# zhengpuas47/ImageAnalysis3

Hardware: AMD Instinct MI355X
Metric: fitted spots/sec (+ FOVs/sec), 2048x2048x50 float32 stack, ~5k spots/FOV (higher is better)
Workload: dtype f64

## Files before the change

### imageanalysis3_amd/csrc/fit.hip

```cpp
#include "ia3_rt.h"
#include "ia3_lm.h"
#include "ia3_init.h"
#include "ia3_kdtree.h"
#include <algorithm>
#include <numeric>
#include <math.h>
#include <string.h>
#include <stddef.h>
#include <time.h>
#include <stdio.h>
#include <stdlib.h>
#include <unistd.h>
#include <mutex>

using namespace ia3;

namespace ia3k {
void kd_build(const double* points, int n, std::vector<ia3::KdNode>& nodes, std::vector<int>& indices, double* mins,
              double* maxes);
}

namespace {

constexpr int SLOTS = 8;
// ... 779 lines not shown
    success_old = LDH(&fa.state[i].success);
    co0 = LDH(&fa.ps[(size_t)i * 11 + 1]); co1 = LDH(&fa.ps[(size_t)i * 11 + 2]); co2 = LDH(&fa.ps[(size_t)i * 11 + 3]);
  }
  const bool ok = n >= NP;
  int nfev = 0, nfev_first = 0;
  const int npass = mode == 2 ? 2 : 1;
#pragma unroll 1
  for (int pass = 0; pass < npass; ++pass) {
    const bool refit = mode == 1 || pass == 1;
    if (pass == 1) { success_old = ok ? 1 : 0; co0 = L->p[1]; co1 = L->p[2]; co2 = L->p[3]; nfev_first = nfev; }
    if (ok) nfev = wave_gaussfit(fa, L, valid, refit ? 2 : (fa.dtype == IA3_F32 ? 0 : 1), c0,
                                 refit ? fa.delta_repeat : fa.delta_first, n, mode == 2 && pass == 0);
  }
  if (mode == 2 && ok && (threadIdx.x & 63) == 0) L->tally[0] += 1ull;
  bool cv = true;
  if (mode != 0 && ok && success_old) {
    const float d0 = co0 - L->p[1], d1 = co1 - L->p[2], d2 = co2 - L->p[3];
    const float dist = (d0 * d0 + d1 * d1) + d2 * d2;
    cv = (double)dist < fa.dist_th2;
  }
  store_result(fa, i, L, mode == 0 ? fa.delta_first : fa.delta_repeat, ok, n, nfev + nfev_first, mode != 0, cv);
  IA3_STAMP(L, 11);
  return cv;
}

constexpr int NCLAIM = 8;
struct StageCtl {
  int n_unconv;
  int abort;
  int ties;
  int stage_reached;
  int pad[28];
  struct Claim { unsigned int next; unsigned int pad[31]; } claim[NCLAIM + 1];
};
static_assert(sizeof(StageCtl) == 128 * (NCLAIM + 2), "one 128-byte line per counter");

__device__ long long d_wait_bound = 1LL << 22;

__device__ __forceinline__ bool wait_done(const int* done, int j, int need, StageCtl* ctl) {
  long long spins = 0;
  for (;;) {
    const int v = __builtin_amdgcn_readfirstlane(__hip_atomic_load(&done[j], __ATOMIC_RELAXED, __HIP_MEMORY_SCOPE_AGENT));
    if (v >= need) { if (spins) __builtin_amdgcn_s_setprio(3); return true; }
    if (spins == 0) __builtin_amdgcn_s_setprio(0);
    if (spins < 256) __builtin_amdgcn_s_sleep(16);
    else if (spins < 1024) __builtin_amdgcn_s_sleep(64);
    else { __builtin_amdgcn_s_sleep(127); __builtin_amdgcn_s_sleep(127); }
    ++spins;
    if ((spins & 15) == 0) {
      const int ab = __builtin_amdgcn_readfirstlane(__hip_atomic_load(&ctl->abort, __ATOMIC_RELAXED, __HIP_MEMORY_SCOPE_AGENT));
      if (spins > d_wait_bound || ab) {
        __hip_atomic_store(&ctl->abort, 1, __ATOMIC_RELAXED, __HIP_MEMORY_SCOPE_AGENT);
        return false;
      }
    }
  }
}

__device__ __forceinline__ void publish(int* done, int i, int value) {
  if ((threadIdx.x & 63) == 0) {
    __builtin_amdgcn_fence(__ATOMIC_RELEASE, "agent");
    asm volatile("s_waitcnt vmcnt(0)" ::: "memory");
    __hip_atomic_fetch_max(&done[i], value, __ATOMIC_RELAXED, __HIP_MEMORY_SCOPE_AGENT);
  }
}

__device__ __forceinline__ void publish_quiet(int* done, int i, int value) {
  if ((threadIdx.x & 63) == 0) __hip_atomic_fetch_max(&done[i], value, __ATOMIC_RELAXED, __HIP_MEMORY_SCOPE_AGENT);
// ... 258 lines not shown
  bool pristine;
  bool first_done;
  StageCtl host_ctl;
  unsigned long long host_counters[5];
  void *d_tie_flag, *d_tie_lost;
  void* kd_block;
  bool ties_resolved;
  bool ties_host = false;
  std::vector<double> host_seeds;
  std::vector<char> kd_stage;
  bool cached;
  std::vector<char> host_stage;
  void* d_snap = nullptr;
};

namespace {

int build_ball(int r, std::vector<signed char>& ball) {
  ball.clear();
  for (int z = -r; z < r; ++z)
    for (int x = -r; x < r; ++x)
      for (int y = -r; y < r; ++y)
        if (z * z + x * x + y * y <= r * r) { ball.push_back((signed char)z); ball.push_back((signed char)x); ball.push_back((signed char)y); ball.push_back(0); }
  return (int)(ball.size() / 4);
}

int g_nb_cap = MAXNB;
int g_fit_fuse = 1;
int g_fit_maxfev = 0;
int g_fit_waves = 2;
int g_fit_merge = 1;
int g_fit_memo = 1;
int g_fit_kdq = KDQ_CAP;

FitArgs make_args(const ia3_fitter* f) {
  FitArgs a;
  a.ims = (const void* const*)f->d_ims; a.fov_of = (const int*)f->d_fov_of; a.fov_start = (const int*)f->d_fov_start;
  a.n_fov = (int)f->ims.size(); a.fov_counters = (unsigned long long*)f->d_fov_counters;
  a.dtype = f->im->dtype; a.Z = f->im->Z; a.X = f->im->X; a.Y = f->im->Y;
  a.n = f->n; a.fuse = g_fit_fuse; a.nb_cap = g_nb_cap; a.nb_r2 = 4.0 * f->prm.radius_fit * (double)f->prm.radius_fit;
  a.seeds = (const double*)f->d_seeds; a.nbr_cnt = (const int*)f->d_nbr_cnt; a.nbr_idx = (const int*)f->d_nbr_idx;
  a.ball = (const int*)f->d_ball; a.nball = f->nball; a.radius = f->prm.radius_fit;
  a.tie_lost = f->ties_resolved ? (const unsigned long long*)f->d_tie_lost : nullptr;
  a.state = (SeedState*)f->d_state; a.ps = (float*)f->d_ps; a.nvox = (int*)f->d_nvox; a.nfev = (int*)f->d_nfev;
  a.memo = g_fit_memo ? (unsigned long long*)f->d_memo : nullptr;
  a.conv = (unsigned char*)f->d_conv; a.n_iter = (int*)f->d_niter; a.counters = (unsigned long long*)f->d_counters;
  a.min_ws = f->prm.min_w * f->prm.min_w; a.max_ws = f->prm.max_w * f->prm.max_w; a.init_w = f->prm.init_w;
  a.delta_first = f->prm.min_delta_center; a.delta_repeat = f->prm.max_delta_center;
  a.dist_th2 = f->prm.max_dist_th * f->prm.max_dist_th;
  a.n_max_iter = f->prm.n_max_iter;
  a.ftol = 1.49012e-8; a.xtol = 1.49012e-8; a.gtol = 0.0; a.maxfev = 1000; a.factor = 100.0;
  if (f->prm.model_variant == 1) {
    a.maxfev = 100 * (NP + 1);
    a.variant = 1;
    for (int k = 0; k < 3; ++k) {
      double w = f->prm.init_w_zxy[k];
      if (w * w > f->prm.max_w || w * w < f->prm.min_w) w = 1.5 * 1.5;
      a.iw[k] = log((a.max_ws - w * w) / (w * w - a.min_ws));
    }
  }
  if (g_fit_maxfev > 0) a.maxfev = g_fit_maxfev;
  return a;
}

}

// ... 162 lines not shown
                       (unsigned long long*)f->d_fov_counters);
  }
  {
    hipError_t le = hipGetLastError();
    if (le != hipSuccess) { ia3_fit_destroy(f); return set_error(IA3_EHIP, "fitter setup launch failed: %s", hipGetErrorString(le)); }
  }
  *out = f;
  return IA3_OK;
}

int ia3_fit_create(const ia3_stack* im, const double* centers_zxy, int n, const ia3_fit_params* p,
                   ia3_fitter** out) {
  if (!im || n < 0 || (n > 0 && !centers_zxy)) return set_error(IA3_EINVAL, "bad argument");
  const FovSeeds one{im, centers_zxy, nullptr, n};
  return fit_create_impl(&one, 1, p, out);
}

}

namespace ia3k {
void set_fit_nblist(int cap) { g_nb_cap = cap < 0 ? 0 : (cap > MAXNB ? MAXNB : cap); }
int get_fit_nblist() { return g_nb_cap; }
void set_fit_fuse(int on) { g_fit_fuse = on ? 1 : 0; }
void set_fit_maxfev(int n) { g_fit_maxfev = n; }
void set_fit_waves(int n) { g_fit_waves = n < 1 ? 1 : (n > IA3_FIT_LB ? IA3_FIT_LB : n); }
void set_fit_merge(int on) { g_fit_merge = on != 0; }
int set_fit_waitbound(int polls) {
  int rc = ia3rt::ensure_init(); if (rc) return rc;
  const long long v = polls > 0 ? (long long)polls : (1LL << 22);
  IA3_HIP(hipMemcpyToSymbol(HIP_SYMBOL(d_wait_bound), &v, sizeof(v)));
  return IA3_OK;
}
void set_fit_memo(int on) { g_fit_memo = on != 0; }
void set_fit_kdq(int cap) { g_fit_kdq = cap < 1 ? 1 : (cap > KDQ_CAP ? KDQ_CAP : cap); }
void fit_host_counters(const ia3_fitter* f, long long out[5]) {
  for (int k = 0; k < 5; ++k) out[k] = (long long)f->host_counters[k];
}
int fit_create_dev(const ia3_stack* im, const double* d_centers_zxy, int n, const ia3_fit_params* p, ia3_fitter** out) {
  if (!im || n < 0 || (n > 0 && !d_centers_zxy)) return set_error(IA3_EINVAL, "bad argument");
  const FovSeeds one{im, nullptr, d_centers_zxy, n};
  return fit_create_impl(&one, 1, p, out);
}
int fit_create_ahead(const ia3_stack* im, const double* d_centers_zxy, int capacity, const unsigned* d_count, int n_cut,
                     const ia3_fit_params* p, ia3_fitter** out) {
  if (!im || capacity < 1 || !d_centers_zxy || !d_count) return set_error(IA3_EINVAL, "bad argument");
  const FovSeeds one{im, nullptr, d_centers_zxy, capacity};
  return fit_create_impl(&one, 1, p, out, d_count, n_cut);
}
int fit_set_count(ia3_fitter* f, int n) {
  if (!f || n < 0 || n > f->n || f->ims.size() != 1) return set_error(IA3_EINVAL, "bad seed count");
  f->n = n;
  f->fov_start.assign({0, n});
  return IA3_OK;
}
int fit_max_fovs() { return MAX_FOV; }
int fit_create_multi(const ia3_stack* const* ims, const double* const* d_centers_zxy, const int* n_seeds, int n_fov,
                     const ia3_fit_params* p, ia3_fitter** out) {
  std::vector<FovSeeds> v((size_t)(n_fov > 0 ? n_fov : 0));
  for (int k = 0; k < n_fov; ++k) v[(size_t)k] = FovSeeds{ims[k], nullptr, d_centers_zxy[k], n_seeds[k]};
  return fit_create_impl(v.data(), n_fov, p, out);
}
int fit_fov_results(ia3_fitter* f, int* n_iter, long long* counters3) {
  const int nf = (int)f->ims.size();
  std::vector<int> it((size_t)nf);
  std::vector<unsigned long long> c(4 * (size_t)nf);
  IA3_HIP(hipStreamSynchronize(stream()));
// ... 15 lines not shown
  hipStream_t st = stream();
  if (fresh) {
    if (!f->pristine) {
      memset(&f->host_ctl, 0, sizeof(StageCtl));
      f->host_ctl.n_unconv = f->n;
      static_assert(offsetof(StageCtl, n_unconv) == 0 && offsetof(StageCtl, abort) == 4, "the first two words are re-armed together");
      IA3_HIP(hipMemcpyAsync(f->d_ctl, &f->host_ctl, 2 * sizeof(int), hipMemcpyHostToDevice, st));
    }
  }
  if (!fresh || !f->pristine)
    IA3_HIP(hipMemsetAsync((char*)f->d_ctl + offsetof(StageCtl, claim), 0, sizeof(StageCtl) - offsetof(StageCtl, claim), st));
  f->pristine = false;
  long long blocks = (long long)(stage1 - stage0) * f->n;
  const long long simds = 4LL * num_cus() * g_fit_waves;
  if (blocks > simds) blocks = simds;
  if (blocks < 1) blocks = 1;
  ProfScope ps(stage0 == 0 ? "fit_first" : "fit_repeat");
  hipLaunchKernelGGL(fit_stages_k, dim3((unsigned)blocks), dim3(64), 0, st, a, f->n, stage0, stage1, (StageCtl*)f->d_ctl,
                     (int*)f->d_done);
  dbg_stamp("fit_stages launched");
  IA3_KCHECK();
  return IA3_OK;
}


__global__ __launch_bounds__(1024) void mail_copy_k(const unsigned* __restrict__ src, unsigned* __restrict__ dst, size_t n4,
                                                    volatile unsigned* seq_word, unsigned seq) {
  const size_t n16 = n4 / 4;
  for (size_t i = threadIdx.x; i < n16; i += 1024) ((uint4*)dst)[i] = ((const uint4*)src)[i];
  for (size_t i = 4 * n16 + threadIdx.x; i < n4; i += 1024) dst[i] = src[i];
  __threadfence_system();
  __syncthreads();
  if (threadIdx.x == 0) *seq_word = seq;
}
static int fetch_block(ia3_fitter* f, bool with_rows) {
  hipStream_t st = stream();
  const size_t head = (size_t)((char*)f->d_ps - (char*)f->d_counters);
  const size_t rows = with_rows ? sizeof(float) * 11 * (size_t)f->n : 0;
  f->host_stage.resize(head + rows);
  void *mh = nullptr, *md = nullptr;
  constexpr size_t MAIL_OFF = 4096;
  constexpr size_t SEQ_OFF = 2048;
  static_assert(sizeof(uint4) == 16, "");
  if (head + rows <= (1u << 20) - MAIL_OFF && (head + rows) % 4 == 0 && ((size_t)f->d_counters & 15) == 0 &&
      host_mailbox(1u << 20, &mh, &md) == IA3_OK) {
    static thread_local unsigned t_seq = 0;
    const unsigned seq = ++t_seq ? t_seq : ++t_seq;
    hipLaunchKernelGGL(mail_copy_k, dim3(1), dim3(1024), 0, st, (const unsigned*)f->d_counters, (unsigned*)((char*)md + MAIL_OFF),
                       (head + rows) / 4, (volatile unsigned*)((char*)md + SEQ_OFF), seq);
    IA3_KCHECK();
    ws_put_deferred_now();
    volatile unsigned* mb = (volatile unsigned*)((char*)mh + SEQ_OFF);
    SpinWait sw;
    while (*mb != seq) {
      sw.relax();
      if (((sw.n & 0xfffff) == 0 || (sw.n > 40400 && (sw.n & 0x3ff) == 0)) && hipStreamQuery(st) != hipErrorNotReady) {
        if (*mb == seq) break;
        IA3_HIP(hipStreamSynchronize(st));
        if (*mb != seq) return set_error(IA3_EHIP, "fit results did not reach the host mailbox");
        break;
      }
    }
    memcpy(f->host_stage.data(), (char*)mh + MAIL_OFF, head + rows);
    return IA3_OK;
  }
  { int rc = stream_wait_spin(st); if (rc) return rc; }
  IA3_HIP(hipMemcpyAsync(f->host_stage.data(), f->d_counters, head + rows, hipMemcpyDeviceToHost, st));
  IA3_HIP(hipStreamSynchronize(st));
  return IA3_OK;
}

static int resolve_ties_host(ia3_fitter* f);
static int resolve_ties(ia3_fitter* f) {
  hipStream_t st = stream();
  const int n = f->n, nf = (int)f->ims.size();
  std::vector<int> flagged((size_t)nf, 1);
  if (f->host_seeds.empty()) {
    f->host_seeds.resize(3 * (size_t)n);
    IA3_HIP(hipMemcpyAsync(f->host_seeds.data(), f->d_seeds, sizeof(double) * 3 * (size_t)n, hipMemcpyDeviceToHost, st));
  }
  IA3_HIP(hipMemcpyAsync(flagged.data(), f->d_fov_ties, sizeof(int) * (size_t)nf, hipMemcpyDeviceToHost, st));
  IA3_HIP(hipStreamSynchronize(st));
// ... 558 lines not shown
```

### imageanalysis3_amd/csrc/gauss.hip

```cpp
#include "ia3_gauss.h"
#include <unistd.h>
#include <cstring>
#include <mutex>

using namespace ia3g;

namespace {

__global__ void border_map_k(int* bmap, int count, int R, int len, int mode) {
  int i = blockIdx.x * 256 + threadIdx.x;
  if (i < count) bmap[i] = border_idx(i - R, len, mode);
}

template <class T, int R, int K, bool TR = false>
__global__ __launch_bounds__(256) void gauss_strided(const T* __restrict__ in, T* __restrict__ out,
                                                     int inner, size_t stride, int len,
                                                     size_t outer_stride, Taps taps,
                                                     const int* __restrict__ bmap, int seg, int cert) {
  constexpr bool FAST = R >= 16;
  constexpr int TQ = (K == 6 || K == 12) ? 24 : ((K == 10) ? 30 : 32);
  static_assert(!TR || TQ % K == 0, "tile must hold whole chunks");
  __shared__ float tile[TR ? 4 : 1][TR ? 64 : 1][TR ? TQ + 1 : 1];
  const int p_raw = blockIdx.x * 256 + threadIdx.x;
  if (!TR && p_raw >= inner) return;
// ... 732 lines not shown
}

using namespace ia3rt;

extern "C" {

int ia3_prepare_depth(int dtype, int Z) {
  int rc = ensure_init(); if (rc) return rc;
  if (dtype != IA3_F32 && dtype != IA3_U16) return set_error(IA3_EINVAL, "dtype");
  return ia3g::column_kernel_source(dtype == IA3_F32, Z);
}
int ia3_set_tuning(int key, int value) {
  if (key == IA3_TUNE_GAUSS_CERT) {
    if (value < -2) return set_error(IA3_EINVAL, "IA3_TUNE_GAUSS_CERT: value must be >= -2");
    g_cert = value;
    return 0;
  }
  if (key == IA3_TUNE_GAUSS_FOLD) { g_fold_on = value != 0; return 0; }
  if (key == IA3_TUNE_DFT_VALU) { ia3k::set_dft_valu(value); return 0; }
  if (key == IA3_TUNE_UPLOAD_THREADS) return ia3rt::set_upload_threads(value);
  if (key == IA3_TUNE_SEED_DENSE) { ia3k::set_seed_dense(value); return 0; }
  if (key == IA3_TUNE_SEED_STRIPS) { ia3k::set_seed_strips(value); return 0; }
  if (key == IA3_TUNE_SEED_FUSED) { ia3k::set_seed_fused(value); return 0; }
  if (key == IA3_TUNE_SEED_SKIP) { ia3k::set_seed_skip(value); return 0; }
  if (key == IA3_TUNE_FIT_NBLIST) { ia3k::set_fit_nblist(value); return 0; }
  if (key == IA3_TUNE_FFT_C2C) { ia3k::set_fft_c2c(value); return 0; }
  if (key == IA3_TUNE_FIT_FUSE) { ia3k::set_fit_fuse(value); return 0; }
  if (key == IA3_TUNE_FIT_WAVES) { ia3k::set_fit_waves(value); return 0; }
  if (key == IA3_TUNE_FIT_MERGE) { ia3k::set_fit_merge(value); return 0; }
  if (key == IA3_TUNE_WARP_ONEPASS) { ia3k::set_warp_onepass(value); return 0; }
  if (key == IA3_TUNE_FIT_KDQ) { ia3k::set_fit_kdq(value); return 0; }
  if (key == IA3_TUNE_FIT_MEMO) { ia3k::set_fit_memo(value); return 0; }
  if (key == IA3_TUNE_COL_RTC) { ia3g::set_column_rtc(value != 0); return 0; }
  if (key == IA3_DEBUG_FIT_MAXFEV) { ia3k::set_fit_maxfev(value); return 0; }
  if (key == IA3_DEBUG_FIT_WAITBOUND) return ia3k::set_fit_waitbound(value);
  return set_error(IA3_EINVAL, "unknown tuning key");
}

static int taps_or_default(double sigma, double truncate, const double* weights, int radius,
                           std::vector<double>& w, int& R) {
  if (weights) {
    if (radius < 0) return set_error(IA3_EINVAL, "negative radius");
    w.assign(weights, weights + 2 * radius + 1);
    R = radius;
  } else {
    if (!(sigma > 0)) return set_error(IA3_EINVAL, "sigma must be > 0");
    gaussian_taps(sigma, truncate, w, R);
  }
  return IA3_OK;
}

int ia3_gaussian_filter_dev(const ia3_stack* im, double sigma, double truncate, int mode,
                            const double* weights, int radius, ia3_stack* out) {
  int rc = ensure_init(); if (rc) return rc;
  if (!im || !out) return set_error(IA3_EINVAL, "null stack");
  if (im->dtype != out->dtype || im->Z != out->Z || im->X != out->X || im->Y != out->Y)
    return set_error(IA3_EINVAL, "input/output stacks differ in shape or dtype");
  if (mode != IA3_MODE_REFLECT && mode != IA3_MODE_NEAREST) return set_error(IA3_EUNSUPPORTED, "mode %d", mode);
  std::vector<double> w; int R;
  rc = taps_or_default(sigma, truncate, weights, radius, w, R); if (rc) return rc;
  Scratch tmp(im->bytes);
  if (!tmp.p) return IA3_ENOMEM;
  if (im->d == out->d) return set_error(IA3_EINVAL, "in-place filtering is not supported");
  return ia3k::gaussian3d(im->d, im->dtype, im->Z, im->X, im->Y, w.data(), R, mode, out->d, tmp.p);
}

// ... 41 lines not shown
```

### imageanalysis3_amd/csrc/ia3_rt.h

```cpp
#pragma once
#include <hip/hip_runtime.h>
#include <stdint.h>
#include <stddef.h>
#include <string>
#include <vector>
#include "../../include/ia3.h"

struct ia3_stack {
  void* d;
  int dtype, Z, X, Y;
  bool owned;
  size_t bytes;
  void* home = nullptr;
};

namespace ia3rt {

int set_error(int code, const char* fmt, ...);
int ensure_init();
hipStream_t stream();
int num_cus();
int host_mailbox(size_t bytes, void** host, void** dev);
int stream_wait_spin(hipStream_t st);
struct SpinWait {
// ... 37 lines not shown
                              hipGetErrorString(_e), __FILE__, __LINE__);                  \
  } while (0)

struct AuxScope {
  bool ok;
  AuxScope();
  ~AuxScope();
};
struct AuxResume {
  bool ok;
  AuxResume();
  ~AuxResume();
};
int aux_join();
struct PutDefer {
  bool outer;
  PutDefer();
  ~PutDefer();
};
void ws_put_deferred_now();
void dbg_stamp(const char* what);

struct ProfScope {
  int slot;
  explicit ProfScope(const char* name);
  ~ProfScope();
};

void gaussian_taps(double sigma, double truncate, std::vector<double>& w, int& radius);

}

namespace ia3k { void set_dft_valu(int on); void set_fft_c2c(int on); void set_seed_dense(int on);
void set_seed_strips(int on); void set_seed_fused(int on); void set_seed_skip(int v); void set_fit_nblist(int cap); void set_fit_fuse(int on); void set_fit_waves(int n); void set_fit_maxfev(int n); void set_fit_merge(int on); void set_warp_onepass(int v); void set_fit_kdq(int cap); void set_fit_memo(int on); int set_fit_waitbound(int polls); }
namespace ia3k {
int gaussian3d(const void* src, int dtype, int Z, int X, int Y, const double* w, int radius, int mode,
               void* dst, void* tmp, int axes = 3);
int highpass_combine(const void* im, const void* low, int dtype, size_t n, void* out);
constexpr int DOG_PAIR_ZGROUPS = 5;
size_t dog_pair_strips(int X, int Y);
int gauss_dog_pair(const void* src, int dtype, int Z, int X, int Y, const double* wf, int rf, const double* wb, int rb,
                   void* dst_front, void* dst_zp, void* tmp, int* forked, float* tmax = nullptr, float* smin = nullptr,
                   float* sabs = nullptr, float* smx = nullptr);
void dog_pair_tiles(int X, int Y, int* ty, int* ntile, size_t* count);
const int* reflect_map(int count, int R, int len);
struct SeedOut {
  std::vector<double> zxyh;
  double th_used;
};
int dog_seed(const ia3_stack* im, const ia3_seed_params& p, SeedOut& out);
struct SeedDev {
  bool on_device = false;
  int n = 0;
  double th_used = 0;
  const double* d_zxy = nullptr;
  const double* d_h = nullptr;
  void* hold = nullptr;
  void (*ahead)(void* ctx, const double* d_zxy, const unsigned* d_count, int max_num_seeds) = nullptr;
  void* ahead_ctx = nullptr;
  SeedOut host;
  ~SeedDev() { if (hold) ia3rt::ws_put(hold); }
};
int dog_seed_dev(const ia3_stack* im, const ia3_seed_params& p, SeedDev& out);
int fit_create_dev(const ia3_stack* im, const double* d_centers_zxy, int n, const ia3_fit_params* p, ia3_fitter** out);
int fit_create_ahead(const ia3_stack* im, const double* d_centers_zxy, int capacity, const unsigned* d_count, int n_cut,
                     const ia3_fit_params* p, ia3_fitter** out);
int fit_set_count(ia3_fitter* f, int n);
// ... 14 lines not shown
```

### imageanalysis3_amd/csrc/seed.hip

```cpp
#include "ia3_rt.h"
#include "ia3_gauss_dev.h"
#include "ia3_seedskip.h"
#include <memory>
#include <algorithm>
#include <math.h>
#include <string.h>
#include <time.h>
#include <stdio.h>
#include <stdlib.h>

namespace {

struct Cand { int z, x, y; float h; };

constexpr int MAXLEV = 64;
struct Levels { double th[MAXLEV]; int n; };

struct SeedCtl {
  unsigned int n_cand;
  unsigned int overflow;
  unsigned int pad[2];
};

template <class T> __device__ __forceinline__ T ldc(const T* p, int z, int x, int y, int X, int Y) {
// ... 791 lines not shown
  __shared__ int chosen_s;
  const unsigned tid = threadIdx.x;
  if (tid < MAXLEV) cnt[tid] = 0;
  if (tid == 0) nk = 0;
  __syncthreads();
  const unsigned n = fin_n(sctl);
  for (unsigned i = tid; i < n; i += 1024) {
    const double h = (double)c[i].h;
    for (int l = 0; l < lev.n; ++l) if (h >= lev.th[l]) atomicAdd(&cnt[l], 1u);
  }
  __syncthreads();
  if (tid == 0) {
    int chosen = lev.n - 1;
    for (int l = 0; l < lev.n; ++l) if ((long long)cnt[l] >= (long long)min_dyn) { chosen = l; break; }
    chosen_s = chosen;
  }
  __syncthreads();
  const double th = lev.th[chosen_s];
  for (unsigned i0 = 0; i0 < n; i0 += 1024) {
    const unsigned i = i0 + tid;
    Cand k{0, 0, 0, 0.f};
    if (i < n) k = c[i];
    const bool keep = i < n && (double)k.h >= th;
    const unsigned long long m = __ballot(keep);
    unsigned base = 0;
    if ((tid & 63) == 0 && m) base = atomicAdd(&nk, (unsigned)__popcll(m));
    base = __shfl(base, 0, 64);
    const unsigned pos = base + (unsigned)__popcll(m & ((1ull << (tid & 63)) - 1ull));
    if (keep && pos < FIN_KEYS) kc[pos] = k;
  }
  __syncthreads();
  const unsigned kept = nk < FIN_KEYS ? nk : FIN_KEYS;
  for (unsigned i = tid; i < kept; i += 1024) { hotcnt[i] = 0u; rank[i] = 0u; }
  if (tid == 0) { fc->chosen = chosen_s; fc->n_kept = nk; fc->n_alive = 0u; fc->done = 0u; }
}
__device__ __forceinline__ unsigned fin_kept(const FinCtl* fc) { return fc->n_kept <= FIN_KEYS ? fc->n_kept : 0u; }

__global__ __launch_bounds__(256) void fin_hot_k(const Cand* __restrict__ kc, const FinCtl* __restrict__ fc, unsigned* __restrict__ hotcnt) {
  __shared__ int tx[256], ty[256];
  const unsigned n = fin_kept(fc);
  if (blockIdx.x * 256 >= n) return;
  const unsigned i = blockIdx.x * 256 + threadIdx.x;
  const int xi = i < n ? kc[i].x : -1, yi = i < n ? kc[i].y : -1;
  const unsigned per = (n + FIN_S - 1) / FIN_S, j0 = blockIdx.y * per, j1 = j0 + per < n ? j0 + per : n;
  unsigned cnt = 0;
  for (unsigned jb = j0; jb < j1; jb += 256) {
    const unsigned j = jb + threadIdx.x;
    __syncthreads();
    tx[threadIdx.x] = j < j1 ? kc[j].x : -2;
    ty[threadIdx.x] = j < j1 ? kc[j].y : -2;
    __syncthreads();
    const unsigned m = j1 - jb < 256 ? j1 - jb : 256;
    for (unsigned t = 0; t < m; ++t) cnt += (tx[t] == xi && ty[t] == yi);
  }
  if (i < n && cnt) atomicAdd(&hotcnt[i], cnt);
}

__global__ __launch_bounds__(256) void fin_rank_k(const Cand* __restrict__ kc, FinCtl* __restrict__ fc, const unsigned* __restrict__ hotcnt,
                                                  int hot_th, unsigned* __restrict__ rank) {
  __shared__ unsigned long long tk[256];
  const unsigned n = fin_kept(fc);
  if (blockIdx.x * 256 >= n) return;
  const unsigned i = blockIdx.x * 256 + threadIdx.x;
  const bool alive = i < n && (hot_th <= 0 || hotcnt[i] < (unsigned)hot_th);
  const unsigned long long ki = i < n ? fin_key(kc[i]) : ~0ull;
  const unsigned per = (n + FIN_S - 1) / FIN_S, j0 = blockIdx.y * per, j1 = j0 + per < n ? j0 + per : n;
  unsigned r = 0;
// ... 4 lines not shown
    tk[threadIdx.x] = aj ? fin_key(kc[j]) : 0ull;
    __syncthreads();
    const unsigned m = j1 - jb < 256 ? j1 - jb : 256;
    for (unsigned t = 0; t < m; ++t) r += tk[t] > ki;
  }
  if (alive) {
    if (r) atomicAdd(&rank[i], r);
    if (blockIdx.y == 0) atomicAdd(&fc->n_alive, 1u);
  }
}

__global__ __launch_bounds__(256) void fin_scatter_k(const SeedCtl* __restrict__ sctl, const Cand* __restrict__ kc, const FinCtl* fc,
                                                     const unsigned* __restrict__ hotcnt, int hot_th, const unsigned* __restrict__ rank,
                                                     int max_num, double* __restrict__ zxy, double* __restrict__ hh, FinCtl* fcw,
                                                     const SeedCtl* __restrict__ lazy, unsigned cap0,
                                                     volatile unsigned* __restrict__ mail, unsigned seq) {
  const unsigned n = fin_kept(fc);
  const unsigned i = blockIdx.x * 256 + threadIdx.x;
  if (i < n) {
    const bool alive = hot_th <= 0 || hotcnt[i] < (unsigned)hot_th;
    const unsigned r = alive ? rank[i] : 0u;
    if (alive && !(max_num > 0 && r >= (unsigned)max_num)) {
      const Cand k = kc[i];
      zxy[3 * r] = k.z; zxy[3 * r + 1] = k.x; zxy[3 * r + 2] = k.y;
      hh[r] = (double)k.h;
    }
  }
  __threadfence();
  __syncthreads();
  if (threadIdx.x != 0) return;
  if (atomicAdd(&fcw->done, 1u) != gridDim.x - 1) return;
  __threadfence();
  const unsigned nc = sctl->n_cand;
  const unsigned ov = sctl->overflow | ((lazy && (lazy->overflow || lazy->n_cand > cap0)) ? 2u : 0u) | (fc->n_kept > FIN_KEYS ? 4u : 0u);
  fcw->n_cand = nc;
  fcw->overflow = ov;
  fcw->pad[0] = lazy ? lazy->pad[0] : 0u;
  if (mail) {
    mail[1] = fcw->n_alive; mail[2] = (unsigned)fcw->chosen; mail[3] = nc; mail[4] = ov;
    mail[5] = fcw->pad[0];
    __threadfence_system();
    mail[0] = seq;
  }
}

}

using namespace ia3rt;

namespace ia3k {

static void finish_seeds(std::vector<Cand>& c, const Levels& lev, const ia3_seed_params& p, int Y,
                         SeedOut& o) {
  int chosen = lev.n - 1;
  for (int i = 0; i < lev.n; ++i) {
    long long cnt = 0;
    for (auto& k : c) cnt += ((double)k.h >= lev.th[i]);
    if (cnt >= (long long)p.min_dynamic_seeds) { chosen = i; break; }
  }
  o.th_used = lev.th[chosen];
  std::vector<Cand> s;
  s.reserve(c.size());
  for (auto& k : c) if ((double)k.h >= lev.th[chosen]) s.push_back(k);
  if (p.remove_hot_pixel && !s.empty()) {
    size_t cap = 64;
    while (cap < 4 * s.size()) cap <<= 1;
    std::vector<long long> keys(cap, -1);
    std::vector<int> cnts(cap, 0);
    auto slot = [&](long long key) {
      size_t h = (size_t)((unsigned long long)key * 0x9E3779B97F4A7C15ull >> 20) & (cap - 1);
      while (keys[h] != -1 && keys[h] != key) h = (h + 1) & (cap - 1);
      return h;
    };
    bool any_hot = false;
    for (auto& k : s) {
      const long long key = (long long)k.x * (Y + 1) + k.y;
      size_t h = slot(key);
      keys[h] = key;
      if (++cnts[h] >= p.hot_pixel_th) any_hot = true;
    }
    if (any_hot) {
      std::vector<Cand> kept;
      kept.reserve(s.size());
      for (auto& k : s) if (cnts[slot((long long)k.x * (Y + 1) + k.y)] < p.hot_pixel_th) kept.push_back(k);
      s.swap(kept);
    }
  }
  std::sort(s.begin(), s.end(), [](const Cand& a, const Cand& b) {
    if (a.h != b.h) return a.h > b.h;
    if (a.z != b.z) return a.z > b.z;
    if (a.x != b.x) return a.x > b.x;
    return a.y > b.y;
  });
  if (p.max_num_seeds > 0 && (size_t)p.max_num_seeds <= s.size()) s.resize(p.max_num_seeds);
  o.zxyh.resize(s.size() * 4);
  for (size_t i = 0; i < s.size(); ++i) {
    o.zxyh[4 * i + 0] = s[i].z; o.zxyh[4 * i + 1] = s[i].x; o.zxyh[4 * i + 2] = s[i].y; o.zxyh[4 * i + 3] = (double)s[i].h;
  }
}

static double now_ms() { struct timespec t; clock_gettime(CLOCK_MONOTONIC, &t); return t.tv_sec * 1e3 + t.tv_nsec * 1e-6; }

int g_strip_bound = 1;
void set_seed_strips(int on) { g_strip_bound = on ? 1 : 0; }
int g_seed_dense = 0;
void set_seed_dense(int on) { g_seed_dense = on ? 1 : 0; }
int g_seed_fused = 1;
void set_seed_fused(int on) { g_seed_fused = on ? 1 : 0; }
int g_seed_skip = 2;
void set_seed_skip(int v) { g_seed_skip = v < 0 ? 0 : (v > 2 ? 2 : v); }
static thread_local double t_skip_run = 0, t_skip_all = 0;

constexpr unsigned LAZY_CAP = 1u << 17;

inline size_t lazy_bound_offset(size_t nb) { return 2 * ((nb + 1) & ~(size_t)1); }
inline double* lazy_bound_ptr(void* bnd, size_t nb) { return (double*)((float*)bnd + lazy_bound_offset(nb)); }
inline size_t lazy_bound_bytes(size_t nb) { return lazy_bound_offset(nb) * sizeof(float) + nb * sizeof(double); }

template <class T>
static void launch_lazy(const void* mx, const void* zp, int Z, int X, int Y, const double* w, int R, int edge,
                        double th_low, void* bnd, Cand0* c0, SeedCtl* ctl0, Cand* out, unsigned capacity, SeedCtl* ctl,
                        hipStream_t s, int stage, const float* smax = nullptr, int sm_ty = 0, int sm_ntile = 0) {
  const int B = R <= 32 ? 32 : 64;
  const int nbx = (X + B - 1) / B, nby = (Y + B - 1) / B;
  const size_t nb = (size_t)Z * nbx * nby;
  float* bmin = (float*)bnd;
  float* babs = bmin + nb;
  double* lb = lazy_bound_ptr(bnd, nb);
  if (stage == 0) {
    ProfScope ps("seed_blockmin");
    constexpr int V = 16 / (int)sizeof(T);
    const bool wide = Y % V == 0 && ((uintptr_t)zp & 15) == 0;
    const int per = 256 * (wide ? V : 1);
    dim3 g((unsigned)((Y + per - 1) / per), (unsigned)nbx, (unsigned)Z);
    if (B == 32 && wide) hipLaunchKernelGGL((blockmin_k<T, 32, V>), g, dim3(256), 0, s, (const T*)zp, Z, X, Y, nbx, nby, bmin, babs);
    else if (B == 32) hipLaunchKernelGGL((blockmin_k<T, 32, 1>), g, dim3(256), 0, s, (const T*)zp, Z, X, Y, nbx, nby, bmin, babs);
    else if (wide) hipLaunchKernelGGL((blockmin_k<T, 64, V>), g, dim3(256), 0, s, (const T*)zp, Z, X, Y, nbx, nby, bmin, babs);
    else hipLaunchKernelGGL((blockmin_k<T, 64, 1>), g, dim3(256), 0, s, (const T*)zp, Z, X, Y, nbx, nby, bmin, babs);
    hipLaunchKernelGGL(blockbound_k, dim3((unsigned)((nb + 255) / 256)), dim3(256), 0, s, (const float*)bmin, (const float*)babs,
// ... 204 lines not shown
    if (fused) {
      const double th_low = th_list;
      const float* sm = (n_strip && g_strip_bound) ? smin_d : nullptr;
      if (im->dtype == IA3_F32) {
        rc = launch_front<float>(tmp2.p, w.data(), Z, X, Y, p.min_edge_distance, th_low, bnd.p, sm, sabs_d, c0buf.as<Cand0>(), dlazy, s, smx_d, skip_sup);
        if (!rc) launch_lazy<float>(nullptr, b.p, Z, X, Y, wb.data(), Rb, p.min_edge_distance, th_low, bnd.p, c0buf.as<Cand0>(), dlazy, dcand, capacity, dctl, s, 2);
      } else {
        rc = launch_front<uint16_t>(tmp2.p, w.data(), Z, X, Y, p.min_edge_distance, th_low, bnd.p, sm, sabs_d, c0buf.as<Cand0>(), dlazy, s, smx_d, skip_sup);
        if (!rc) launch_lazy<uint16_t>(nullptr, b.p, Z, X, Y, wb.data(), Rb, p.min_edge_distance, th_low, bnd.p, c0buf.as<Cand0>(), dlazy, dcand, capacity, dctl, s, 2);
      }
      if (rc) return rc;
    } else if (lazy) {
      if (im->dtype == IA3_F32)
        launch_lazy<float>(maxim, b.p, Z, X, Y, wb.data(), Rb, p.min_edge_distance, th_low, bnd.p, c0buf.as<Cand0>(), dlazy, dcand, capacity, dctl, s, 1,
                           paired ? smaxbuf.as<float>() : nullptr, sm_ty, sm_ntile);
      else
        launch_lazy<uint16_t>(maxim, b.p, Z, X, Y, wb.data(), Rb, p.min_edge_distance, th_low, bnd.p, c0buf.as<Cand0>(), dlazy, dcand, capacity, dctl, s, 1,
                              paired ? smaxbuf.as<float>() : nullptr, sm_ty, sm_ntile);
    } else {
      ProfScope ps("seed_detect");
      if (im->dtype == IA3_F32)
        launch_detect<float>(p.filt_size, maxim, minim, Z, X, Y, p.min_edge_distance, th_low, dcand, capacity, dctl, s);
      else
        launch_detect<uint16_t>(p.filt_size, maxim, minim, Z, X, Y, p.min_edge_distance, th_low, dcand, capacity, dctl, s);
    }
    IA3_KCHECK();
    if (dev_finish && attempt == 0) {
      char* fb = (char*)fin;
      hipError_t fe;
      FinCtl* fc = (FinCtl*)fb;
      const int hot_th = p.remove_hot_pixel ? p.hot_pixel_th : 0;
      void *mail_host = nullptr, *mail_dev = nullptr;
      static thread_local unsigned t_seq = 0;
      const unsigned seq = ++t_seq ? t_seq : ++t_seq;
      if (host_mailbox(64, &mail_host, &mail_dev) != IA3_OK) { mail_host = mail_dev = nullptr; }
      {
        ProfScope pf("seed_finish");
        unsigned* hot = (unsigned*)(fb + o_hot);
        unsigned* rank = (unsigned*)(fb + o_rank);
        Cand* kc = (Cand*)(fb + o_kc);
        hipLaunchKernelGGL(fin_levels_k, dim3(1), dim3(1024), 0, s, (const SeedCtl*)dctl, (const Cand*)dcand, lev, p.min_dynamic_seeds, fc, kc, hot, rank);
        if (hot_th > 0)
          hipLaunchKernelGGL(fin_hot_k, dim3(FIN_KEYS / 256, FIN_S), dim3(256), 0, s, (const Cand*)kc, (const FinCtl*)fc, hot);
        hipLaunchKernelGGL(fin_rank_k, dim3(FIN_KEYS / 256, FIN_S), dim3(256), 0, s, (const Cand*)kc, fc, (const unsigned*)hot, hot_th, rank);
        hipLaunchKernelGGL(fin_scatter_k, dim3(FIN_KEYS / 256), dim3(256), 0, s, (const SeedCtl*)dctl, (const Cand*)kc, (const FinCtl*)fc,
                           (const unsigned*)hot, hot_th, (const unsigned*)rank, p.max_num_seeds, (double*)(fb + o_zxy), (double*)(fb + o_h), fc,
                           lazy ? (const SeedCtl*)dlazy : (const SeedCtl*)nullptr, LAZY_CAP, (volatile unsigned*)mail_dev, seq);
      }
      FinCtl hfc;
      fe = hipGetLastError();
      dbg_stamp("seed stage queued");
      if (fe == hipSuccess && dev->ahead) dev->ahead(dev->ahead_ctx, (const double*)(fb + o_zxy), (const unsigned*)&fc->n_alive, p.max_num_seeds);
      if (fe == hipSuccess && mail_host) {
        volatile unsigned* mb = (volatile unsigned*)mail_host;
        SpinWait sw;
        while (mb[0] != seq) {
          sw.relax();
          if (((sw.n & 0xfffff) == 0 || (sw.n > 40400 && (sw.n & 0x3ff) == 0)) && hipStreamQuery(s) != hipErrorNotReady) {
            if (mb[0] == seq) break;
            fe = hipStreamSynchronize(s);
            if (fe == hipSuccess && mb[0] != seq) fe = hipErrorUnknown;
            break;
          }
        }
        hfc.n_alive = mb[1]; hfc.chosen = (int)mb[2]; hfc.n_cand = mb[3]; hfc.overflow = mb[4];
        if (fused) t_skip_run = (double)mb[5];
        dbg_stamp("seed count seen");
      } else {
        if (fe == hipSuccess) fe = hipMemcpyAsync(&hfc, fc, sizeof(FinCtl), hipMemcpyDeviceToHost, s);
        if (fe == hipSuccess) fe = hipStreamSynchronize(s);
        if (fe == hipSuccess && fused) t_skip_run = (double)hfc.pad[0];
      }
      if (fe != hipSuccess) return set_error(IA3_EHIP, "seed finish failed: %s", hipGetErrorString(fe));
      if (hfc.overflow & 2u)
        return dog_seed_impl(im, p, out, dev, true);
      if (top_list && hfc.chosen != 0)
        return dog_seed_impl(im, p, out, dev, force_dense, true);
      hctl.n_cand = hfc.n_cand; hctl.overflow = hfc.overflow;
      if (hctl.n_cand <= FIN_CAP && !hctl.overflow) {
        int n = (int)hfc.n_alive;
        if (p.max_num_seeds > 0 && p.max_num_seeds <= n) n = p.max_num_seeds;
        dev->on_device = true;
        dev->n = n;
        dev->th_used = lev.th[hfc.chosen];
        dev->d_zxy = (const double*)(fb + o_zxy);
        dev->d_h = (const double*)(fb + o_h);
        dev->hold = fin;
        fin = nullptr;
        if (dbg) fprintf(stderr, "dog_seed: device finish, %u candidates -> %d seeds\n", hctl.n_cand, n);
        return IA3_OK;
      }
      ws_put(fin);
      fin = nullptr;
    }
    hbuf.resize(HDR + (size_t)FIRST * sizeof(Cand));
    IA3_HIP(hipMemcpyAsync(hbuf.data(), bp, hbuf.size(), hipMemcpyDeviceToHost, s));
    IA3_HIP(hipStreamSynchronize(s));
    memcpy(&hctl, hbuf.data(), sizeof(SeedCtl));
    memcpy(&hlazy, hbuf.data() + sizeof(SeedCtl), sizeof(SeedCtl));
    if (fused) t_skip_run = (double)hlazy.pad[0];
    if (lazy && (hlazy.overflow || hlazy.n_cand > LAZY_CAP)) return dog_seed_impl(im, p, out, dev, true);
    if (hctl.n_cand <= capacity) {
      cand.resize(hctl.n_cand);
      const unsigned nfirst = hctl.n_cand < FIRST ? hctl.n_cand : FIRST;
// ... 269 lines not shown
```

### include/ia3.h

```cpp
#ifndef IA3_H
#define IA3_H

#include <stdint.h>

#ifdef __cplusplus
extern "C" {
#endif

#define IA3_U16 0
#define IA3_F32 1

#define IA3_OK 0
#define IA3_EINVAL (-1)
#define IA3_EHIP (-2)
#define IA3_ENOMEM (-3)
#define IA3_ECAPACITY (-4)
#define IA3_EUNSUPPORTED (-5)

#define IA3_MODE_REFLECT 0
#define IA3_MODE_NEAREST 1
#define IA3_MODE_CONSTANT 2

typedef struct ia3_stack ia3_stack;

int ia3_init(int device);
const char* ia3_last_error(void);
const char* ia3_version(void);
int ia3_device_name(char* buf, int len);
int ia3_sync(void);
void* ia3_stream(void);
int ia3_release_workspace(void);
int ia3_prepare_depth(int dtype, int Z);
int ia3_workspace_stats(double* out6);
int ia3_seed_skip_stats(double* out2);
int ia3_profile_enable(int on);
int ia3_profile_collect(char* buf, int len);
#define IA3_TUNE_GAUSS_CERT 1
#define IA3_TUNE_DFT_VALU 2
#define IA3_TUNE_UPLOAD_THREADS 3
#define IA3_TUNE_SEED_DENSE 4
#define IA3_TUNE_FIT_NBLIST 5
#define IA3_TUNE_FFT_C2C 6
#define IA3_TUNE_FIT_FUSE 7
#define IA3_TUNE_GAUSS_FOLD 8
#define IA3_TUNE_SEED_STRIPS 9
#define IA3_TUNE_FIT_WAVES 10
#define IA3_TUNE_FIT_MERGE 11
#define IA3_TUNE_WARP_ONEPASS 12
#define IA3_TUNE_FIT_KDQ 13
#define IA3_TUNE_FIT_MEMO 14
#define IA3_TUNE_SEED_FUSED 15
#define IA3_TUNE_SEED_SKIP 16
#define IA3_TUNE_COL_RTC 17
#define IA3_DEBUG_FIT_MAXFEV 100
#define IA3_DEBUG_FIT_WAITBOUND 101
int ia3_set_tuning(int key, int value);

int ia3_stack_upload(const void* host, int dtype, int Z, int X, int Y, ia3_stack** out);
int ia3_stack_alloc(int dtype, int Z, int X, int Y, ia3_stack** out);
int ia3_stack_load_file(const char* path, long long offset_bytes, int frames, int X, int Y, int big_endian,
                        ia3_stack** out);
int ia3_stack_wrap(void* devptr, int dtype, int Z, int X, int Y, ia3_stack** out);
int ia3_stack_deinterleave(const ia3_stack* raw, int start, int step, int Z, ia3_stack** out);
int ia3_buffer_upload(const void* host, size_t bytes, void** devptr);
void ia3_buffer_free(void* devptr);
int ia3_buffer_alloc(size_t bytes, void** devptr);
int ia3_buffer_download(const void* devptr, size_t bytes, void* host);
int ia3_stack_download(const ia3_stack* s, void* host);
int ia3_stack_info(const ia3_stack* s, int* dtype, int* Z, int* X, int* Y, void** devptr);
void ia3_stack_free(ia3_stack* s);

int ia3_gaussian_filter(const void* im, int dtype, int Z, int X, int Y, double sigma, double truncate,
                        int mode, const double* weights, int radius, void* out);
int ia3_gaussian_filter_dev(const ia3_stack* im, double sigma, double truncate, int mode,
                            const double* weights, int radius, ia3_stack* out);

int ia3_gaussian_highpass(const void* im, int dtype, int Z, int X, int Y, double sigma, double truncate,
                          const double* weights, int radius, void* out);
int ia3_gaussian_highpass_dev(const ia3_stack* im, double sigma, double truncate,
                              const double* weights, int radius, ia3_stack* out);

int ia3_remove_hot_pixels(const void* im, int dtype, int Z, int X, int Y, double hot_pix_th, double hot_th,
                          void* out, int* n_hot);

int ia3_z_shift_correction(const void* im, int dtype, int Z, int X, int Y, void* out_u16, float* medians_out);
int ia3_illumination_correct(const void* im_u16, int Z, int X, int Y, const void* profile, int prof_dtype,
// ... 238 lines not shown
```

Before: 2.712 million.

## Fuse seed-finish level/hot-pixel passes into one packed kernel; multi-block mailbox copy

Adds fin_pack_k, a single-block kernel that picks the threshold level, counts hot pixels in a shared-memory hash table and compacts the kept candidates in one launch. It replaces the fin_levels_k plus fin_hot_k pair, and on overflow the host retries with the old path. Separately, the fitter's mailbox copy to pinned host memory now runs across 16 blocks, with a ticket counter deciding which block publishes the sequence word, instead of one block. Both aim to shorten small serial tail kernels on the critical path. The cost is extra complexity, a possible second pass when the pack capacity overflows, and shared-memory pressure from the 128KB hash table.

```diff
diff --git a/imageanalysis3_amd/csrc/fit.hip b/imageanalysis3_amd/csrc/fit.hip
--- a/imageanalysis3_amd/csrc/fit.hip
+++ b/imageanalysis3_amd/csrc/fit.hip
@@ -835,8 +835,9 @@
   int stage_reached;
   int pad[28];
   struct Claim { unsigned int next; unsigned int pad[31]; } claim[NCLAIM + 1];
+  Claim mail;
 };
-static_assert(sizeof(StageCtl) == 128 * (NCLAIM + 2), "one 128-byte line per counter");
+static_assert(sizeof(StageCtl) == 128 * (NCLAIM + 3), "one 128-byte line per counter");
 
 __device__ long long d_wait_bound = 1LL << 22;
 
@@ -1161,6 +1162,7 @@
 int g_fit_merge = 1;
 int g_fit_memo = 1;
 int g_fit_kdq = KDQ_CAP;
+int g_fit_mail = 1;
 
 FitArgs make_args(const ia3_fitter* f) {
   FitArgs a;
@@ -1389,6 +1391,7 @@
   return IA3_OK;
 }
 void set_fit_memo(int on) { g_fit_memo = on != 0; }
+void set_fit_mail(int on) { g_fit_mail = on != 0; }
 void set_fit_kdq(int cap) { g_fit_kdq = cap < 1 ? 1 : (cap > KDQ_CAP ? KDQ_CAP : cap); }
 void fit_host_counters(const ia3_fitter* f, long long out[5]) {
   for (int k = 0; k < 5; ++k) out[k] = (long long)f->host_counters[k];
@@ -1470,6 +1473,20 @@
   __threadfence_system();
   __syncthreads();
   if (threadIdx.x == 0) *seq_word = seq;
+}
+constexpr unsigned MAIL_BLOCKS = 16;
+__global__ __launch_bounds__(1024) void mail_copy_grid_k(const unsigned* src, unsigned* __restrict__ dst, size_t n4,
+                                                         volatile unsigned* seq_word, unsigned seq, unsigned* ticket) {
+  const size_t n16 = n4 / 4, t = (size_t)blockIdx.x * 1024 + threadIdx.x, step = (size_t)gridDim.x * 1024;
+  for (size_t i = t; i < n16; i += step) ((uint4*)dst)[i] = ((const uint4*)src)[i];
+  for (size_t i = 4 * n16 + t; i < n4; i += step) dst[i] = src[i];
+  __threadfence_system();
+  __syncthreads();
+  if (threadIdx.x != 0) return;
+  if (atomicAdd(ticket, 1u) != gridDim.x - 1) return;
+  __threadfence_system();
+  __hip_atomic_store(ticket, 0u, __ATOMIC_RELAXED, __HIP_MEMORY_SCOPE_AGENT);
+  *seq_word = seq;
 }
 static int fetch_block(ia3_fitter* f, bool with_rows) {
   hipStream_t st = stream();
@@ -1484,8 +1501,12 @@
       host_mailbox(1u << 20, &mh, &md) == IA3_OK) {
     static thread_local unsigned t_seq = 0;
     const unsigned seq = ++t_seq ? t_seq : ++t_seq;
-    hipLaunchKernelGGL(mail_copy_k, dim3(1), dim3(1024), 0, st, (const unsigned*)f->d_counters, (unsigned*)((char*)md + MAIL_OFF),
-                       (head + rows) / 4, (volatile unsigned*)((char*)md + SEQ_OFF), seq);
+    if (g_fit_mail)
+      hipLaunchKernelGGL(mail_copy_grid_k, dim3(MAIL_BLOCKS), dim3(1024), 0, st, (const unsigned*)f->d_counters, (unsigned*)((char*)md + MAIL_OFF),
+                         (head + rows) / 4, (volatile unsigned*)((char*)md + SEQ_OFF), seq, &((StageCtl*)f->d_ctl)->mail.next);
+    else
+      hipLaunchKernelGGL(mail_copy_k, dim3(1), dim3(1024), 0, st, (const unsigned*)f->d_counters, (unsigned*)((char*)md + MAIL_OFF),
+                         (head + rows) / 4, (volatile unsigned*)((char*)md + SEQ_OFF), seq);
     IA3_KCHECK();
     ws_put_deferred_now();
     volatile unsigned* mb = (volatile unsigned*)((char*)mh + SEQ_OFF);
diff --git a/imageanalysis3_amd/csrc/gauss.hip b/imageanalysis3_amd/csrc/gauss.hip
--- a/imageanalysis3_amd/csrc/gauss.hip
+++ b/imageanalysis3_amd/csrc/gauss.hip
@@ -788,6 +788,8 @@
   if (key == IA3_TUNE_FIT_KDQ) { ia3k::set_fit_kdq(value); return 0; }
   if (key == IA3_TUNE_FIT_MEMO) { ia3k::set_fit_memo(value); return 0; }
   if (key == IA3_TUNE_COL_RTC) { ia3g::set_column_rtc(value != 0); return 0; }
+  if (key == IA3_TUNE_SEED_FINISH) { ia3k::set_seed_finish(value); return 0; }
+  if (key == IA3_TUNE_FIT_MAIL) { ia3k::set_fit_mail(value); return 0; }
   if (key == IA3_DEBUG_FIT_MAXFEV) { ia3k::set_fit_maxfev(value); return 0; }
   if (key == IA3_DEBUG_FIT_WAITBOUND) return ia3k::set_fit_waitbound(value);
   return set_error(IA3_EINVAL, "unknown tuning key");
diff --git a/imageanalysis3_amd/csrc/ia3_rt.h b/imageanalysis3_amd/csrc/ia3_rt.h
--- a/imageanalysis3_amd/csrc/ia3_rt.h
+++ b/imageanalysis3_amd/csrc/ia3_rt.h
@@ -93,7 +93,7 @@
 }
 
 namespace ia3k { void set_dft_valu(int on); void set_fft_c2c(int on); void set_seed_dense(int on);
-void set_seed_strips(int on); void set_seed_fused(int on); void set_seed_skip(int v); void set_fit_nblist(int cap); void set_fit_fuse(int on); void set_fit_waves(int n); void set_fit_maxfev(int n); void set_fit_merge(int on); void set_warp_onepass(int v); void set_fit_kdq(int cap); void set_fit_memo(int on); int set_fit_waitbound(int polls); }
+void set_seed_strips(int on); void set_seed_fused(int on); void set_seed_skip(int v); void set_fit_nblist(int cap); void set_fit_fuse(int on); void set_fit_waves(int n); void set_fit_maxfev(int n); void set_fit_merge(int on); void set_warp_onepass(int v); void set_fit_kdq(int cap); void set_fit_memo(int on); int set_fit_waitbound(int polls); void set_seed_finish(int v); void set_fit_mail(int on); }
 namespace ia3k {
 int gaussian3d(const void* src, int dtype, int Z, int X, int Y, const double* w, int radius, int mode,
                void* dst, void* tmp, int axes = 3);
diff --git a/imageanalysis3_amd/csrc/seed.hip b/imageanalysis3_amd/csrc/seed.hip
--- a/imageanalysis3_amd/csrc/seed.hip
+++ b/imageanalysis3_amd/csrc/seed.hip
@@ -847,7 +847,7 @@
   __syncthreads();
   const unsigned kept = nk < FIN_KEYS ? nk : FIN_KEYS;
   for (unsigned i = tid; i < kept; i += 1024) { hotcnt[i] = 0u; rank[i] = 0u; }
-  if (tid == 0) { fc->chosen = chosen_s; fc->n_kept = nk; fc->n_alive = 0u; fc->done = 0u; }
+  if (tid == 0) { fc->chosen = chosen_s; fc->n_kept = nk; fc->n_alive = 0u; fc->done = 0u; fc->pad[1] = 0u; }
 }
 __device__ __forceinline__ unsigned fin_kept(const FinCtl* fc) { return fc->n_kept <= FIN_KEYS ? fc->n_kept : 0u; }
 
@@ -918,7 +918,7 @@
   if (atomicAdd(&fcw->done, 1u) != gridDim.x - 1) return;
   __threadfence();
   const unsigned nc = sctl->n_cand;
-  const unsigned ov = sctl->overflow | ((lazy && (lazy->overflow || lazy->n_cand > cap0)) ? 2u : 0u) | (fc->n_kept > FIN_KEYS ? 4u : 0u);
+  const unsigned ov = sctl->overflow | ((lazy && (lazy->overflow || lazy->n_cand > cap0)) ? 2u : 0u) | (fc->n_kept > FIN_KEYS ? 4u : 0u) | (fc->pad[1] ? 8u : 0u);
   fcw->n_cand = nc;
   fcw->overflow = ov;
   fcw->pad[0] = lazy ? lazy->pad[0] : 0u;
@@ -928,6 +928,83 @@
     __threadfence_system();
     mail[0] = seq;
   }
+}
+
+constexpr unsigned PACK_CAP = 8192;
+constexpr unsigned PACK_SLOTS = 16384;
+constexpr unsigned PACK_EMPTY = 0xffffffffu;
+__device__ __forceinline__ unsigned pack_hash(unsigned key) { return (key * 0x9E3779B9u) >> 18; }
+static_assert(PACK_SLOTS == 1u << 14 && PACK_CAP * 2 <= PACK_SLOTS && PACK_CAP <= FIN_KEYS, "table geometry");
+
+__global__ __launch_bounds__(1024) void fin_pack_k(const SeedCtl* __restrict__ sctl, const Cand* __restrict__ c, Levels lev,
+                                                   int min_dyn, int hot_th, int Y, unsigned cap, FinCtl* __restrict__ fc,
+                                                   Cand* __restrict__ kc, unsigned* __restrict__ rank) {
+  __shared__ unsigned tkey[PACK_SLOTS], tcnt[PACK_SLOTS];
+  __shared__ unsigned cnt[MAXLEV];
+  __shared__ unsigned nk;
+  __shared__ int chosen_s;
+  const unsigned tid = threadIdx.x, lane = tid & 63;
+  if (tid < MAXLEV) cnt[tid] = 0;
+  if (tid == 0) nk = 0;
+  if (hot_th > 0)
+    for (unsigned q = tid; q < PACK_SLOTS; q += 1024) { tkey[q] = PACK_EMPTY; tcnt[q] = 0u; }
+  __syncthreads();
+  const unsigned n = fin_n(sctl);
+  for (unsigned i0 = 0; i0 < n; i0 += 1024) {
+    const unsigned i = i0 + tid;
+    const double h = i < n ? (double)c[i].h : 0.0;
+    for (int l = 0; l < lev.n; ++l) {
+      const unsigned long long m = __ballot(i < n && h >= lev.th[l]);
+      if (lane == 0 && m) atomicAdd(&cnt[l], (unsigned)__popcll(m));
+    }
+  }
+  __syncthreads();
+  if (tid == 0) {
+    int chosen = lev.n - 1;
+    for (int l = 0; l < lev.n; ++l) if ((long long)cnt[l] >= (long long)min_dyn) { chosen = l; break; }
+    chosen_s = chosen;
+  }
+  __syncthreads();
+  const unsigned npass = cnt[chosen_s];
+  if (npass > cap) {
+    if (tid == 0) { fc->chosen = chosen_s; fc->n_kept = 0u; fc->n_alive = 0u; fc->done = 0u; fc->pad[1] = 1u; }
+    return;
+  }
+  const double th = lev.th[chosen_s];
+  if (hot_th > 0) {
+    for (unsigned i = tid; i < n; i += 1024) {
+      const Cand k = c[i];
+      if (!((double)k.h >= th)) continue;
+      const unsigned key = (unsigned)k.x * (unsigned)(Y + 1) + (unsigned)k.y;
+      for (unsigned s = pack_hash(key);; s = (s + 1) & (PACK_SLOTS - 1)) {
+        const unsigned was = atomicCAS(&tkey[s], PACK_EMPTY, key);
+        if (was == PACK_EMPTY || was == key) { atomicAdd(&tcnt[s], 1u); break; }
+      }
+    }
+    __syncthreads();
+  }
+  for (unsigned i0 = 0; i0 < n; i0 += 1024) {
+    const unsigned i = i0 + tid;
+    Cand k{0, 0, 0, 0.f};
+    if (i < n) k = c[i];
+    bool keep = i < n && (double)k.h >= th;
+    if (keep && hot_th > 0) {
+      const unsigned key = (unsigned)k.x * (unsigned)(Y + 1) + (unsigned)k.y;
+      unsigned s = pack_hash(key);
+      while (tkey[s] != key) s = (s + 1) & (PACK_SLOTS - 1);
+      keep = tcnt[s] < (unsigned)hot_th;
+    }
+    const unsigned long long m = __ballot(keep);
+    unsigned base = 0;
+    if (lane == 0 && m) base = atomicAdd(&nk, (unsigned)__popcll(m));
+    base = __shfl(base, 0, 64);
+    const unsigned pos = base + (unsigned)__popcll(m & ((1ull << lane) - 1ull));
+    if (keep) kc[pos] = k;
+  }
+  __syncthreads();
+  const unsigned kept = nk;
+  for (unsigned i = tid; i < kept; i += 1024) rank[i] = 0u;
+  if (tid == 0) { fc->chosen = chosen_s; fc->n_kept = kept; fc->n_alive = 0u; fc->done = 0u; fc->pad[1] = 0u; }
 }
 
 }
@@ -991,6 +1068,8 @@
 void set_seed_strips(int on) { g_strip_bound = on ? 1 : 0; }
 int g_seed_dense = 0;
 void set_seed_dense(int on) { g_seed_dense = on ? 1 : 0; }
+int g_seed_finish = 1;
+void set_seed_finish(int v) { g_seed_finish = v < 0 ? 0 : v; }
 int g_seed_fused = 1;
 void set_seed_fused(int on) { g_seed_fused = on ? 1 : 0; }
 int g_seed_skip = 2;
@@ -1261,44 +1340,53 @@
       const int hot_th = p.remove_hot_pixel ? p.hot_pixel_th : 0;
       void *mail_host = nullptr, *mail_dev = nullptr;
       static thread_local unsigned t_seq = 0;
-      const unsigned seq = ++t_seq ? t_seq : ++t_seq;
       if (host_mailbox(64, &mail_host, &mail_dev) != IA3_OK) { mail_host = mail_dev = nullptr; }
-      {
-        ProfScope pf("seed_finish");
-        unsigned* hot = (unsigned*)(fb + o_hot);
-        unsigned* rank = (unsigned*)(fb + o_rank);
-        Cand* kc = (Cand*)(fb + o_kc);
-        hipLaunchKernelGGL(fin_levels_k, dim3(1), dim3(1024), 0, s, (const SeedCtl*)dctl, (const Cand*)dcand, lev, p.min_dynamic_seeds, fc, kc, hot, rank);
-        if (hot_th > 0)
-          hipLaunchKernelGGL(fin_hot_k, dim3(FIN_KEYS / 256, FIN_S), dim3(256), 0, s, (const Cand*)kc, (const FinCtl*)fc, hot);
-        hipLaunchKernelGGL(fin_rank_k, dim3(FIN_KEYS / 256, FIN_S), dim3(256), 0, s, (const Cand*)kc, fc, (const unsigned*)hot, hot_th, rank);
-        hipLaunchKernelGGL(fin_scatter_k, dim3(FIN_KEYS / 256), dim3(256), 0, s, (const SeedCtl*)dctl, (const Cand*)kc, (const FinCtl*)fc,
-                           (const unsigned*)hot, hot_th, (const unsigned*)rank, p.max_num_seeds, (double*)(fb + o_zxy), (double*)(fb + o_h), fc,
-                           lazy ? (const SeedCtl*)dlazy : (const SeedCtl*)nullptr, LAZY_CAP, (volatile unsigned*)mail_dev, seq);
-      }
       FinCtl hfc;
-      fe = hipGetLastError();
-      dbg_stamp("seed stage queued");
-      if (fe == hipSuccess && dev->ahead) dev->ahead(dev->ahead_ctx, (const double*)(fb + o_zxy), (const unsigned*)&fc->n_alive, p.max_num_seeds);
-      if (fe == hipSuccess && mail_host) {
-        volatile unsigned* mb = (volatile unsigned*)mail_host;
-        SpinWait sw;
-        while (mb[0] != seq) {
-          sw.relax();
-          if (((sw.n & 0xfffff) == 0 || (sw.n > 40400 && (sw.n & 0x3ff) == 0)) && hipStreamQuery(s) != hipErrorNotReady) {
-            if (mb[0] == seq) break;
-            fe = hipStreamSynchronize(s);
-            if (fe == hipSuccess && mb[0] != seq) fe = hipErrorUnknown;
-            break;
+      const unsigned pack_cap = g_seed_finish <= 0 ? 0u : (g_seed_finish == 1 || (unsigned)g_seed_finish > PACK_CAP ? PACK_CAP : (unsigned)g_seed_finish);
+      for (bool packed = pack_cap > 0;; packed = false) {
+        const unsigned seq = ++t_seq ? t_seq : ++t_seq;
+        {
+          ProfScope pf("seed_finish");
+          unsigned* hot = (unsigned*)(fb + o_hot);
+          unsigned* rank = (unsigned*)(fb + o_rank);
+          Cand* kc = (Cand*)(fb + o_kc);
+          if (packed) {
+            hipLaunchKernelGGL(fin_pack_k, dim3(1), dim3(1024), 0, s, (const SeedCtl*)dctl, (const Cand*)dcand, lev, p.min_dynamic_seeds, hot_th, Y, pack_cap, fc, kc, rank);
+          } else {
+            hipLaunchKernelGGL(fin_levels_k, dim3(1), dim3(1024), 0, s, (const SeedCtl*)dctl, (const Cand*)dcand, lev, p.min_dynamic_seeds, fc, kc, hot, rank);
+            if (hot_th > 0)
+              hipLaunchKernelGGL(fin_hot_k, dim3(FIN_KEYS / 256, FIN_S), dim3(256), 0, s, (const Cand*)kc, (const FinCtl*)fc, hot);
           }
+          const int hot_rank = packed ? 0 : hot_th;
+          hipLaunchKernelGGL(fin_rank_k, dim3(FIN_KEYS / 256, FIN_S), dim3(256), 0, s, (const Cand*)kc, fc, (const unsigned*)hot, hot_rank, rank);
+          hipLaunchKernelGGL(fin_scatter_k, dim3(FIN_KEYS / 256), dim3(256), 0, s, (const SeedCtl*)dctl, (const Cand*)kc, (const FinCtl*)fc,
+                             (const unsigned*)hot, hot_rank, (const unsigned*)rank, p.max_num_seeds, (double*)(fb + o_zxy), (double*)(fb + o_h), fc,
+                             lazy ? (const SeedCtl*)dlazy : (const SeedCtl*)nullptr, LAZY_CAP, (volatile unsigned*)mail_dev, seq);
         }
-        hfc.n_alive = mb[1]; hfc.chosen = (int)mb[2]; hfc.n_cand = mb[3]; hfc.overflow = mb[4];
-        if (fused) t_skip_run = (double)mb[5];
-        dbg_stamp("seed count seen");
-      } else {
-        if (fe == hipSuccess) fe = hipMemcpyAsync(&hfc, fc, sizeof(FinCtl), hipMemcpyDeviceToHost, s);
-        if (fe == hipSuccess) fe = hipStreamSynchronize(s);
-        if (fe == hipSuccess && fused) t_skip_run = (double)hfc.pad[0];
+        fe = hipGetLastError();
+        dbg_stamp("seed stage queued");
+        if (fe == hipSuccess && dev->ahead) dev->ahead(dev->ahead_ctx, (const double*)(fb + o_zxy), (const unsigned*)&fc->n_alive, p.max_num_seeds);
+        if (fe == hipSuccess && mail_host) {
+          volatile unsigned* mb = (volatile unsigned*)mail_host;
+          SpinWait sw;
+          while (mb[0] != seq) {
+            sw.relax();
+            if (((sw.n & 0xfffff) == 0 || (sw.n > 40400 && (sw.n & 0x3ff) == 0)) && hipStreamQuery(s) != hipErrorNotReady) {
+              if (mb[0] == seq) break;
+              fe = hipStreamSynchronize(s);
+              if (fe == hipSuccess && mb[0] != seq) fe = hipErrorUnknown;
+              break;
+            }
+          }
+          hfc.n_alive = mb[1]; hfc.chosen = (int)mb[2]; hfc.n_cand = mb[3]; hfc.overflow = mb[4];
+          if (fused) t_skip_run = (double)mb[5];
+          dbg_stamp("seed count seen");
+        } else {
+          if (fe == hipSuccess) fe = hipMemcpyAsync(&hfc, fc, sizeof(FinCtl), hipMemcpyDeviceToHost, s);
+          if (fe == hipSuccess) fe = hipStreamSynchronize(s);
+          if (fe == hipSuccess && fused) t_skip_run = (double)hfc.pad[0];
+        }
+        if (fe != hipSuccess || !packed || !(hfc.overflow & 8u)) break;
       }
       if (fe != hipSuccess) return set_error(IA3_EHIP, "seed finish failed: %s", hipGetErrorString(fe));
       if (hfc.overflow & 2u)
diff --git a/include/ia3.h b/include/ia3.h
--- a/include/ia3.h
+++ b/include/ia3.h
@@ -52,6 +52,8 @@
 #define IA3_TUNE_SEED_FUSED 15
 #define IA3_TUNE_SEED_SKIP 16
 #define IA3_TUNE_COL_RTC 17
+#define IA3_TUNE_SEED_FINISH 18
+#define IA3_TUNE_FIT_MAIL 19
 #define IA3_DEBUG_FIT_MAXFEV 100
 #define IA3_DEBUG_FIT_WAITBOUND 101
 int ia3_set_tuning(int key, int value);
diff --git a/profiles/r05_tail/timed_steps.py b/profiles/r05_tail/timed_steps.py
--- /dev/null
+++ b/profiles/r05_tail/timed_steps.py
@@ -0,0 +1,24 @@
+import csv, sys, collections, re
+path, nsteps = sys.argv[1], int(sys.argv[2])
+rows = list(csv.DictReader(open(path)))
+rows.sort(key=lambda r: int(r["Start_Timestamp"]))
+def short(n):
+    n = n.replace("(anonymous namespace)::", "").replace("void ", "")
+    n = re.sub(r"\(.*$", "", n)
+    return n
+starts = [i for i, r in enumerate(rows) if "seed_front_k" in r["Kernel_Name"]]
+marks = [i for i, r in enumerate(rows) if "gauss_axis0_folded" in r["Kernel_Name"]]
+marks = marks[-nsteps:]
+first = marks[0]
+sel = rows[first:]
+agg = collections.OrderedDict()
+for r in sel:
+    k = short(r["Kernel_Name"])
+    agg.setdefault(k, []).append((int(r["End_Timestamp"]) - int(r["Start_Timestamp"])) / 1e3)
+print("| kernel | launches per step | avg us | us per step |")
+print("|---|---|---|---|")
+tot = 0
+for k, v in agg.items():
+    print("| `%s` | %.1f | %.1f | %.1f |" % (k, len(v) / nsteps, sum(v) / len(v), sum(v) / nsteps)); tot += sum(v) / nsteps
+span = (int(sel[-1]["End_Timestamp"]) - int(sel[0]["Start_Timestamp"])) / 1e3 / nsteps
+print("kernel time per step %.1f us; span per step %.1f us (incl. the gap to the next step for all but the last)" % (tot, span))
```

Result: slower. 2.615 million (-3.6%).
